# gaspachoo/EEG2Video

Measured on AMD Instinct MI355X. Metric: 6-frame 288x512 clips/sec (50-step DDIM), higher is better.
Workload: dtype f32; 1 GPU; 1xMI355X: batch=8/GPU synthetic latents [B,4,6,36,64] + [B,77,768] cond, 50-step DDIM, CFG 12.5, 288x512x6 VAE decode, fp32 (BASELINE configs[1]); clips_per_gpu=8, ddim_steps=50, unet_samples_per_ddim_step=16, weights=random-init SD-v1-4 architecture, counter RNG seed 42/43, collective=none

## Files before the change

### eeg2video_amd/csrc/attn.hip

```cpp
#include "h16.h"
#include "kernels.h"
#include "prof.h"
#include "runtime.h"
#include "act_io.h"

#include <cstdlib>
#include <type_traits>

namespace e2v {

typedef float f32x16 __attribute__((ext_vector_type(16)));
typedef float f32x4 __attribute__((ext_vector_type(4)));

struct AttnBlock { int qb, head, sf; bool valid; };
__host__ __device__ __forceinline__ int attn_xcd_unit(const int n, const int F, const int heads) {
    return n % 8 == 0 ? 0 : (n * F) % 8 == 0 ? 1 : 2;
}
__device__ __forceinline__ AttnBlock attn_block_of(const AttnArgs& p, const int nqb) {
    const int b = blockIdx.x, xcd = b & 7, idx = b >> 3;
    const int S = p.n * p.F;
    const int unit = attn_xcd_unit(p.n, p.F, p.heads);
    AttnBlock r;
    if (unit == 0) {
        const int per = p.F * p.heads * nqb;
        const int ul = idx / per, w = idx - ul * per;
        const int smp = ul * 8 + xcd;
        const int f = w / (p.heads * nqb), w2 = w - f * (p.heads * nqb);
        r.sf = smp * p.F + f; r.head = w2 / nqb; r.qb = w2 - r.head * nqb; r.valid = smp < p.n;
    } else if (unit == 1) {
        const int per = p.heads * nqb;
        const int ul = idx / per, w = idx - ul * per;
        r.sf = ul * 8 + xcd; r.head = w / nqb; r.qb = w - r.head * nqb; r.valid = r.sf < S;
    } else {
        const int ul = idx / nqb;
        const int pair = ul * 8 + xcd;
        r.qb = idx - ul * nqb; r.sf = pair / p.heads; r.head = pair - r.sf * p.heads; r.valid = pair < S * p.heads;
    }
    return r;
}
__device__ __forceinline__ AttnBlock attn_block(const AttnArgs& p) { return attn_block_of(p, (p.Nq + 127) / 128); }
static inline unsigned attn_grid_of(const AttnArgs& a, const unsigned nqb) {
    const int unit = attn_xcd_unit(a.n, a.F, a.heads);
    if (unit == 0) return 8u * (a.n / 8) * (unsigned)(a.F * a.heads) * nqb;
    if (unit == 1) return 8u * ((a.n * a.F) / 8) * (unsigned)a.heads * nqb;
    return 8u * ((a.n * a.F * a.heads + 7) / 8) * nqb;
}
static inline unsigned attn_grid(const AttnArgs& a) { return attn_grid_of(a, (a.Nq + 127) / 128); }

std::string attn_shape_tag(const AttnArgs& a) {
    return " D" + std::to_string(a.D) + " Nq" + std::to_string(a.Nq) + " Nk" + std::to_string(a.Nk) + " n" + std::to_string(a.n) + " F" + std::to_string(a.F) +
           " h" + std::to_string(a.heads);
}

template <int D>
__global__ __launch_bounds__(256) void flash_attn_kernel(const AttnArgs p) {
    constexpr int LD = D + 4;
    constexpr int TF = D / 32;
    constexpr bool VREM = (D - 32 * TF) == 8;
    constexpr int T = VREM ? TF : (D + 31) / 32;
    constexpr int TA = T > 0 ? T : 1;
    constexpr int G = D / 8;
    constexpr int DQ = D / 4;
    constexpr int KT = 32;
    constexpr int NF4 = KT * DQ;
    constexpr int LPT = (NF4 + 255) / 256;
    extern __shared__ __attribute__((aligned(16))) float smem[];

    const int tid = threadIdx.x;
    const int lane = tid & 63, wave = tid >> 6;
    const int j = lane & 31, h = lane >> 5;
    const AttnBlock blk = attn_block(p);
    if (!blk.valid) return;
    const int sf = blk.sf;
    const int smp = sf / p.F, f = sf - smp * p.F;
    const int head = blk.head;
    const int q0 = (blk.qb * 4 + wave) * 32;
    const bool active = q0 < p.Nq;

    int nseg = 1;
    size_t kvbase[2];
    if (p.mode == 0) {
        kvbase[0] = (size_t)(smp * p.F) * p.Nk;
        kvbase[1] = (size_t)(smp * p.F + (f > 0 ? f - 1 : 0)) * p.Nk;
        nseg = f >= 2 ? 2 : 1;
    } else {
        kvbase[0] = kvbase[1] = (size_t)smp * p.Nk;
    }
    const int tps = (p.Nk + KT - 1) / KT;
    const int ntiles = nseg * tps;

    f32x4 qf[G];
    {
        const int qrow = min(q0 + j, p.Nq - 1);
        const float* qp = p.q + ((size_t)sf * p.Nq + qrow) * p.ldq + head * D + h * 4;
        const float c = p.scale * 1.44269504088896340736f;
#pragma unroll
        for (int g = 0; g < G; ++g) {
            qf[g] = *reinterpret_cast<const f32x4*>(qp + g * 8);
            qf[g] *= c;
        }
    }

    constexpr unsigned OOB = 0x80000000u;
    auto rsrc_of = [](const void* ptr) {
        const unsigned long long v = reinterpret_cast<unsigned long long>(ptr);
        const unsigned lo = __builtin_amdgcn_readfirstlane((unsigned)v);
        const unsigned hi = __builtin_amdgcn_readfirstlane((unsigned)(v >> 32));
        return __builtin_amdgcn_make_buffer_rsrc(reinterpret_cast<void*>(((unsigned long long)hi << 32) | lo), (short)0, 0x7FFFFFF0,
                                                 0x00020000);
    };
    int ld_row[LPT];
    unsigned ld_off[LPT];
#pragma unroll
    for (int e = 0; e < LPT; ++e) {
        const int idx = tid + 256 * e;
        const int row = idx / DQ, c4 = idx - row * DQ;
        ld_row[e] = row;
        ld_off[e] = idx < NF4 ? (unsigned)(row * p.ldkv + c4 * 4) * 4u : OOB;
    }
    f32x4 kreg[LPT], vreg[LPT];
    auto load_tile = [&](int tt) {
        const int seg = tt / tps;
        const int key0 = (tt - seg * tps) * KT;
        const size_t first = (kvbase[seg] + key0) * p.ldkv + head * D;
        const __amdgpu_buffer_rsrc_t rk = rsrc_of(p.k + first), rv = rsrc_of(p.v + first);
        const int left = p.Nk - key0;
#pragma unroll
        for (int e = 0; e < LPT; ++e) {
            unsigned off = ld_off[e];
            if (left < KT) off = ld_row[e] < left ? off : OOB;
            kreg[e] = __builtin_bit_cast(f32x4, __builtin_amdgcn_raw_buffer_load_b128(rk, off, 0, 0));
            vreg[e] = __builtin_bit_cast(f32x4, __builtin_amdgcn_raw_buffer_load_b128(rv, off, 0, 0));
        }
    };
    auto store_tile = [&](int buf) {
        float* Ks = smem + buf * (2 * KT * LD);
        float* Vs = Ks + KT * LD;
#pragma unroll
        for (int e = 0; e < LPT; ++e) {
            const int idx = tid + 256 * e;
            if (idx < NF4) {
                const int row = idx / DQ, c4 = idx - row * DQ;
                *reinterpret_cast<f32x4*>(Ks + row * LD + c4 * 4) = kreg[e];
                *reinterpret_cast<f32x4*>(Vs + row * LD + c4 * 4) = vreg[e];
            }
        }
    };

    f32x16 acc[TA];
#pragma unroll
    for (int t = 0; t < TA; ++t)
#pragma unroll
        for (int r = 0; r < 16; ++r) acc[t][r] = 0.f;
    f32x4 rem0 = {0.f, 0.f, 0.f, 0.f}, rem1 = {0.f, 0.f, 0.f, 0.f};
    float m_i = -INFINITY, l_i = 0.f;

    load_tile(0);
    store_tile(0);
    __syncthreads();

    for (int tt = 0; tt < ntiles; ++tt) {
        const int buf = tt & 1;
        if (tt + 1 < ntiles) load_tile(tt + 1);
        const int seg_c = tt / tps;
        const int kbase = (tt - seg_c * tps) * KT;
        auto tile_body = [&](const int key0, const int sub, auto ragged) {
            const float* Ks = smem + buf * (2 * KT * LD) + sub * 32 * LD;
            const float* Vs = smem + buf * (2 * KT * LD) + KT * LD + sub * 32 * LD;
            const f32x16 zero16 = {0.f, 0.f, 0.f, 0.f, 0.f, 0.f, 0.f, 0.f, 0.f, 0.f, 0.f, 0.f, 0.f, 0.f, 0.f, 0.f};
            f32x16 st;
            const float* kp = Ks + j * LD + h * 4;
#pragma unroll
            for (int g = 0; g < G; ++g) {
                const f32x4 kf = *reinterpret_cast<const f32x4*>(kp + g * 8);
#pragma unroll
                for (int s = 0; s < 4; ++s)
                    st = __builtin_amdgcn_mfma_f32_32x32x2f32(kf[s], qf[g][s], (g == 0 && s == 0) ? zero16 : st, 0, 0, 0);
            }
            if constexpr (decltype(ragged)::value) {
#pragma unroll
                for (int r = 0; r < 16; ++r) {
                    const int key = key0 + (r & 3) + 8 * (r >> 2) + 4 * h;
                    if (key >= p.Nk) st[r] = -INFINITY;
                }
            }
            float mt = st[0];
#pragma unroll
            for (int r = 1; r < 16; ++r) mt = __builtin_fmaxf(mt, st[r]);
            mt = __builtin_fmaxf(mt, __shfl_xor(mt, 32));
            const float m_new = __builtin_fmaxf(m_i, mt);
            const bool moved = __any(m_new > m_i);
            float ps = 0.f;
#pragma unroll
            for (int r = 0; r < 16; ++r) {
                st[r] = __builtin_amdgcn_exp2f(st[r] - m_new);
                ps += st[r];
            }
            float alpha = 1.0f;
            if (moved) {
                alpha = __builtin_amdgcn_exp2f(m_i - m_new);
                l_i *= alpha;
            }
            l_i += ps;
            m_i = m_new;
#pragma unroll
            for (int t = 0; t < T; ++t) {
                if (moved) {
#pragma unroll
                    for (int r = 0; r < 16; ++r) acc[t][r] *= alpha;
                }
                const int dv = min(t * 32 + j, D - 1);
                const float* vp = Vs + (4 * h) * LD + dv;
#pragma unroll
                for (int r = 0; r < 16; ++r) {
                    const float vv = vp[((r & 3) + 8 * (r >> 2)) * LD];
                    acc[t] = __builtin_amdgcn_mfma_f32_32x32x2f32(vv, st[r], acc[t], 0, 0, 0);
                }
            }
            if constexpr (VREM) {
                if (moved) {
                    rem0 *= alpha;
                    rem1 *= alpha;
                }
                const float* vr = Vs + (4 * h) * LD + 32 * TF;
#pragma unroll
                for (int r = 0; r < 16; ++r) {
                    const float* row = vr + ((r & 3) + 8 * (r >> 2)) * LD;
                    const f32x4 v0 = *reinterpret_cast<const f32x4*>(row);
                    const f32x4 v1 = *reinterpret_cast<const f32x4*>(row + 4);
                    rem0 += v0 * st[r];
                    rem1 += v1 * st[r];
                }
            }
        };
#pragma unroll
        for (int sub = 0; sub < KT / 32; ++sub) {
            const int key0 = kbase + 32 * sub;
            if (active && key0 < p.Nk) {
                if (key0 + 32 <= p.Nk) tile_body(key0, sub, std::false_type{});
                else tile_body(key0, sub, std::true_type{});
            }
        }
        if (tt + 1 < ntiles) store_tile(buf ^ 1);
        __syncthreads();
    }

    const float l_tot = l_i + __shfl_xor(l_i, 32);
    if constexpr (VREM) {
#pragma unroll
        for (int e = 0; e < 4; ++e) {
            rem0[e] += __shfl_xor(rem0[e], 32);
            rem1[e] += __shfl_xor(rem1[e], 32);
        }
    }
    if (active && q0 + j < p.Nq) {
        const float inv = 1.0f / l_tot;
        float* op = p.o + ((size_t)sf * p.Nq + q0 + j) * p.ldo + head * D;
#pragma unroll
        for (int t = 0; t < T; ++t)
#pragma unroll
            for (int rg = 0; rg < 4; ++rg) {
                const int dv = t * 32 + 8 * rg + 4 * h;
                if (dv < D) {
                    f32x4 o;
#pragma unroll
                    for (int e = 0; e < 4; ++e) o[e] = acc[t][rg * 4 + e] * inv;
                    *reinterpret_cast<f32x4*>(op + dv) = o;
                }
            }
        if constexpr (VREM) {
            const f32x4 o = (h ? rem1 : rem0) * inv;
            *reinterpret_cast<f32x4*>(op + 32 * TF + 4 * h) = o;
        }
    }
}

typedef __bf16 abf16x4 __attribute__((ext_vector_type(4)));
typedef __bf16 abf16x8 __attribute__((ext_vector_type(8)));

template <typename H, int D, bool FOLD, int KT>
__global__ __launch_bounds__(256) void flash_attn_b16io_kernel(const AttnArgs p) {
    constexpr int DP = (D + 15) / 16 * 16;
    constexpr int KS = DP / 16;
    constexpr int T = (D + 31) / 32;
    constexpr int KROW = DP * 2 + 16;
    constexpr int VROW = ((T * 16) % 32 == 16) ? T * 64 : T * 64 + 64;
    constexpr int KBYTES = KT * KROW, VBYTES = KT * VROW;
    constexpr int STAGE = (KBYTES + VBYTES + 15) / 16 * 16;
    constexpr bool SUMV = (D % 32) != 0;
    constexpr int LROW = D % 32, LREG = 4 * (LROW / 8) + (LROW & 3), LHALF = (LROW >> 2) & 1;
    constexpr int C8 = D / 8;
    constexpr int NP = KT * C8;
    constexpr int LPT = (NP + 255) / 256;
    extern __shared__ __attribute__((aligned(16))) char smem_h[];

    const int tid = threadIdx.x;
    const int lane = tid & 63, wave = tid >> 6;
    const int j = lane & 31, h = lane >> 5;
    const AttnBlock blk = attn_block(p);
    if (!blk.valid) return;
    const int sf = blk.sf;
    const int smp = sf / p.F, f = sf - smp * p.F;
    const int head = blk.head;
    const int q0 = (blk.qb * 4 + wave) * 32;
    const bool active = q0 < p.Nq;
    const H* __restrict__ Q = reinterpret_cast<const H*>(p.q);
    const H* __restrict__ K = reinterpret_cast<const H*>(p.k);
    const H* __restrict__ V = reinterpret_cast<const H*>(p.v);

    int nseg = 1;
    size_t kvbase[2];
    if (p.mode == 0) {
        kvbase[0] = (size_t)(smp * p.F) * p.Nk;
        kvbase[1] = (size_t)(smp * p.F + (f > 0 ? f - 1 : 0)) * p.Nk;
        nseg = f >= 2 ? 2 : 1;
    } else {
        kvbase[0] = kvbase[1] = (size_t)smp * p.Nk;
    }
    const int tps = (p.Nk + KT - 1) / KT;
    const int ntiles = nseg * tps;

    for (int i = tid * 16; i < 2 * STAGE; i += 256 * 16)
        *reinterpret_cast<f32x4*>(smem_h + i) = f32x4{0.f, 0.f, 0.f, 0.f};
    if constexpr (SUMV) {
        __syncthreads();
        if (tid < 2 * KT)
            *reinterpret_cast<H*>(smem_h + (tid / KT) * STAGE + KBYTES + (tid % KT) * VROW + D * 2) = (H)1.0f;
    }

    hx8<H> qf[KS];
    {
        const int qrow = min(q0 + j, p.Nq - 1);
        const H* qp = Q + ((size_t)sf * p.Nq + qrow) * p.ldq + head * D;
#pragma unroll
        for (int s = 0; s < KS; ++s) {
            const int k0 = 16 * s + 8 * h;
            hx8<H> a;
#pragma unroll
            for (int e = 0; e < 8; ++e) a[e] = (H)0.f;
            if (k0 < D) a = *reinterpret_cast<const hx8<H>*>(qp + k0);
            if constexpr (FOLD) {
                const float qs = p.scale * 1.44269504088896340736f;
#pragma unroll
                for (int e = 0; e < 8; ++e) a[e] = (H)((float)a[e] * qs);
            }
            qf[s] = a;
        }
    }
    const float sc = p.scale * 1.44269504088896340736f;
    __syncthreads();

    constexpr unsigned OOB = 0x80000000u;
    auto rsrc_of = [](const void* ptr) {
        const unsigned long long v = reinterpret_cast<unsigned long long>(ptr);
        const unsigned lo = __builtin_amdgcn_readfirstlane((unsigned)v);
        const unsigned hi = __builtin_amdgcn_readfirstlane((unsigned)(v >> 32));
        return __builtin_amdgcn_make_buffer_rsrc(reinterpret_cast<void*>(((unsigned long long)hi << 32) | lo), (short)0, 0x7FFFFFF0,
                                                 0x00020000);
    };
    int ld_row[LPT], ld_c8[LPT];
    unsigned ld_off[LPT];
#pragma unroll
    for (int e = 0; e < LPT; ++e) {
        const int idx = tid + 256 * e;
        const int row = idx / C8, c8 = idx - row * C8;
        ld_row[e] = row; ld_c8[e] = c8;
        ld_off[e] = idx < NP ? (unsigned)(row * p.ldkv + c8 * 8) * 2u : OOB;
    }
    f32x4 kreg[LPT], vreg[LPT];
    auto load_tile = [&](const int seg, const int key0) {
        const size_t first = (kvbase[seg] + key0) * p.ldkv + head * D;
        const __amdgpu_buffer_rsrc_t rk = rsrc_of(K + first), rv = rsrc_of(V + first);
        const int left = p.Nk - key0;
#pragma unroll
        for (int e = 0; e < LPT; ++e) {
            unsigned off = ld_off[e];
            if (left < KT) off = ld_row[e] < left ? off : OOB;
            kreg[e] = __builtin_bit_cast(f32x4, __builtin_amdgcn_raw_buffer_load_b128(rk, off, 0, 0));
            vreg[e] = __builtin_bit_cast(f32x4, __builtin_amdgcn_raw_buffer_load_b128(rv, off, 0, 0));
        }
    };
    auto store_tile = [&](int buf) {
        char* Kl = smem_h + buf * STAGE;
        char* Vl = Kl + KBYTES;
#pragma unroll
        for (int e = 0; e < LPT; ++e) {
            if (tid + 256 * e < NP) {
                *reinterpret_cast<f32x4*>(Kl + ld_row[e] * KROW + ld_c8[e] * 16) = kreg[e];
                *reinterpret_cast<f32x4*>(Vl + ld_row[e] * VROW + ld_c8[e] * 16) = vreg[e];
            }
        }
    };

    f32x16 acc[T];
#pragma unroll
    for (int t = 0; t < T; ++t)
#pragma unroll
        for (int r = 0; r < 16; ++r) acc[t][r] = 0.f;
    float m_i = -INFINITY, l_i = 0.f;
    f32x16 negm;
#pragma unroll
    for (int r = 0; r < 16; ++r) negm[r] = 0.f;

    load_tile(0, 0);
    store_tile(0);
    __syncthreads();

    const int ti = lane & 15;
    const int tr_off = (4 * h + (ti >> 2)) * VROW + (16 * ((lane >> 4) & 1) + 4 * (ti & 3)) * 2;

    int key0 = 0;
    for (int tt = 0; tt < ntiles; ++tt) {
        const int buf = tt & 1;
        if (tt == tps) key0 = 0;
        if (tt + 1 < ntiles) {
            if (tt + 1 == tps) load_tile(1, 0); else load_tile(tt + 1 > tps ? 1 : 0, key0 + KT);
        }
#pragma unroll
        for (int sub = 0; sub < KT / 32; ++sub) {
        const int keyb = key0 + 32 * sub;
        if (active && keyb < p.Nk) {
            const char* Kl = smem_h + buf * STAGE + sub * 32 * KROW;
            const char* Vl = smem_h + buf * STAGE + KBYTES + sub * 32 * VROW;
            const f32x16 zero16 = {0.f, 0.f, 0.f, 0.f, 0.f, 0.f, 0.f, 0.f, 0.f, 0.f, 0.f, 0.f, 0.f, 0.f, 0.f, 0.f};
            f32x16 st;
            const char* kp = Kl + j * KROW + h * 16;
#pragma unroll
            for (int s = 0; s < KS; ++s) {
                const hx8<H> kf = *reinterpret_cast<const hx8<H>*>(kp + s * 32);
                st = mfma_32x32x16(kf, qf[s], s == 0 ? (FOLD ? negm : zero16) : st);
            }
            if (keyb + 32 > p.Nk) {
                asm volatile("" ::: "memory");
#pragma unroll
                for (int r = 0; r < 16; ++r) {
                    const int key = keyb + (r & 3) + 8 * (r >> 2) + 4 * h;
                    if (key >= p.Nk) st[r] = -INFINITY;
                }
            }
            float mt = st[0];
#pragma unroll
            for (int r = 1; r < 16; ++r) mt = __builtin_fmaxf(mt, st[r]);
            float alpha = 1.0f;
            bool moved;
            if constexpr (FOLD) {
                {
                    float a = mt, b = mt;
                    asm volatile("s_nop 1\n\tv_permlane32_swap_b32 %0, %1" : "+v"(a), "+v"(b));
                    mt = __builtin_fmaxf(a, b);
                }
                constexpr float DEFER = 8.0f;
                const bool first = tt == 0 && sub == 0;
                const float d = first ? mt : (mt > DEFER ? mt : 0.f);
                moved = __any(d != 0.f);
                if (moved) {
                    asm volatile("" ::: "memory");
                    alpha = first ? 1.0f : __builtin_amdgcn_exp2f(-d);
#pragma unroll
                    for (int r = 0; r < 16; ++r) { st[r] -= d; negm[r] -= d; }
                }
#pragma unroll
                for (int r = 0; r < 16; ++r) st[r] = __builtin_amdgcn_exp2f(st[r]);
            } else {
                mt = __builtin_fmaxf(mt, __shfl_xor(mt, 32)) * sc;
                const float m_new = __builtin_fmaxf(m_i, mt);
                moved = __any(m_new > m_i);
                float ps = 0.f;
#pragma unroll
                for (int r = 0; r < 16; ++r) {
                    st[r] = __builtin_amdgcn_exp2f(__builtin_fmaf(st[r], sc, -m_new));
                    if constexpr (!SUMV) ps += st[r];
                }
                if (moved) {
                    alpha = __builtin_amdgcn_exp2f(m_i - m_new);
                    if constexpr (!SUMV) l_i *= alpha;
                }
                if constexpr (!SUMV) l_i += ps;
                m_i = m_new;
            }
            if constexpr (FOLD && !SUMV) {
                float ps = 0.f;
#pragma unroll
                for (int r = 0; r < 16; ++r) ps += st[r];
                l_i = l_i * alpha + ps;
            }
            hx8<H> pf[2];
#pragma unroll
            for (int s = 0; s < 2; ++s)
#pragma unroll
                for (int e = 0; e < 8; ++e) pf[s][e] = (H)st[8 * s + e];
#pragma unroll
            for (int t = 0; t < T; ++t) {
                if (moved) {
                    asm volatile("" ::: "memory");
#pragma unroll
                    for (int r = 0; r < 16; ++r) acc[t][r] *= alpha;
                }
                const char* vb = Vl + tr_off + t * 64;
#pragma unroll
                for (int s = 0; s < 2; ++s) {
                    const hx4<H> lo = lds_read_tr16<H>((vb + (16 * s) * VROW));
                    const hx4<H> hi = lds_read_tr16<H>((vb + (16 * s + 8) * VROW));
                    const hx8<H> vf = __builtin_shufflevector(lo, hi, 0, 1, 2, 3, 4, 5, 6, 7);
                    acc[t] = mfma_32x32x16(vf, pf[s], acc[t]);
                }
            }
        }
        }
        if (tt + 1 < ntiles) store_tile(buf ^ 1);
        __syncthreads();
        key0 += KT;
    }

    float l_tot;
    if constexpr (SUMV) l_tot = __shfl(acc[T - 1][LREG], j + 32 * LHALF);
    else l_tot = l_i + __shfl_xor(l_i, 32);
    if (active && q0 + j < p.Nq) {
        const float inv = 1.0f / l_tot;
        H* op = reinterpret_cast<H*>(p.o) + ((size_t)sf * p.Nq + q0 + j) * p.ldo + head * D;
#pragma unroll
        for (int t = 0; t < T; ++t)
#pragma unroll
            for (int rg = 0; rg < 4; ++rg) {
                const int dv = t * 32 + 8 * rg + 4 * h;
                if (dv < D) {
                    hx4<H> o;
#pragma unroll
                    for (int e = 0; e < 4; ++e) o[e] = (H)(acc[t][rg * 4 + e] * inv);
                    *reinterpret_cast<hx4<H>*>(op + dv) = o;
                }
            }
    }
}

template <typename H, int D>
__global__ __launch_bounds__(256) void cross_attn_resident_kernel(const AttnArgs p, const int tpw, const int chunks) {
    constexpr int DP = (D + 15) / 16 * 16;
    constexpr int KS = DP / 16;
    constexpr int T = (D + 31) / 32;
    constexpr int KROW = DP * 2 + 16;
    constexpr int VROW = ((T * 16) % 32 == 16) ? T * 64 : T * 64 + 64;
    constexpr int NKT = 3, NKEY = 32 * NKT;
    constexpr int KBYTES = NKEY * KROW;
    constexpr bool SUMV = (D % 32) != 0;
    constexpr int LROW = D % 32, LREG = 4 * (LROW / 8) + (LROW & 3), LHALF = (LROW >> 2) & 1;
    constexpr int C8 = D / 8;
    extern __shared__ __attribute__((aligned(16))) char smem_c[];

    const int tid = threadIdx.x;
    const int lane = tid & 63, wave = tid >> 6;
    const int j = lane & 31, h = lane >> 5;
    const int b = blockIdx.x, xcd = b & 7, idx = b >> 3;
    int smp, head, chunk;
    if (p.n % 8 == 0) {
        const int per = p.heads * chunks;
// ... 1126 lines not shown
```

Baseline: 0.5995 clips/s.

## Restructure flash-attention tile loop and use permlane swaps and MFMA for remainder

Reworks the flash-attention main loop so buffer indices are compile-time constant in an unrolled pair of steps, and tracks segment and key offsets incrementally instead of dividing each iteration. Replaces cross-half __shfl_xor reductions with v_permlane32_swap via inline asm, hoists the alpha rescale into a single branch, and computes the D%32==8 remainder with 4x4x1 MFMAs instead of vector FMAs. The aim is to cut per-tile index arithmetic, LDS-based shuffles and VALU work. The inline asm relies on gfx950-specific permlane semantics, and the 4x4 MFMA remainder mapping must match the original output layout.

```diff
diff --git a/eeg2video_amd/csrc/attn.hip b/eeg2video_amd/csrc/attn.hip
--- a/eeg2video_amd/csrc/attn.hip
+++ b/eeg2video_amd/csrc/attn.hip
@@ -52,6 +52,11 @@
            " h" + std::to_string(a.heads);
 }
 
+__device__ __forceinline__ void half_pair(const float x, float& lo, float& hi) {
+    lo = x; hi = x;
+    asm volatile("s_nop 1\n\tv_permlane32_swap_b32 %0, %1" : "+v"(lo), "+v"(hi));
+}
+
 template <int D>
 __global__ __launch_bounds__(256) void flash_attn_kernel(const AttnArgs p) {
     constexpr int LD = D + 4;
@@ -119,9 +124,7 @@
         ld_off[e] = idx < NF4 ? (unsigned)(row * p.ldkv + c4 * 4) * 4u : OOB;
     }
     f32x4 kreg[LPT], vreg[LPT];
-    auto load_tile = [&](int tt) {
-        const int seg = tt / tps;
-        const int key0 = (tt - seg * tps) * KT;
+    auto load_tile = [&](const int seg, const int key0) {
         const size_t first = (kvbase[seg] + key0) * p.ldkv + head * D;
         const __amdgpu_buffer_rsrc_t rk = rsrc_of(p.k + first), rv = rsrc_of(p.v + first);
         const int left = p.Nk - key0;
@@ -155,102 +158,120 @@
     f32x4 rem0 = {0.f, 0.f, 0.f, 0.f}, rem1 = {0.f, 0.f, 0.f, 0.f};
     float m_i = -INFINITY, l_i = 0.f;
 
-    load_tile(0);
+    auto tile_body = [&](const int buf, const int key0, const bool ragged) {
+        const float* Ks = smem + buf * (2 * KT * LD);
+        const float* Vs = Ks + KT * LD;
+        const f32x16 zero16 = {0.f, 0.f, 0.f, 0.f, 0.f, 0.f, 0.f, 0.f, 0.f, 0.f, 0.f, 0.f, 0.f, 0.f, 0.f, 0.f};
+        f32x16 st;
+        const float* kp = Ks + j * LD + h * 4;
+#pragma unroll
+        for (int g = 0; g < G; ++g) {
+            const f32x4 kf = *reinterpret_cast<const f32x4*>(kp + g * 8);
+#pragma unroll
+            for (int s = 0; s < 4; ++s)
+                st = __builtin_amdgcn_mfma_f32_32x32x2f32(kf[s], qf[g][s], (g == 0 && s == 0) ? zero16 : st, 0, 0, 0);
+        }
+        if (ragged) {
+            asm volatile("" ::: "memory");
+#pragma unroll
+            for (int r = 0; r < 16; ++r) {
+                const int key = key0 + (r & 3) + 8 * (r >> 2) + 4 * h;
+                if (key >= p.Nk) st[r] = -INFINITY;
+            }
+        }
+        float mt = st[0];
+#pragma unroll
+        for (int r = 1; r < 16; ++r) mt = __builtin_fmaxf(mt, st[r]);
+        {
+            float lo, hi;
+            half_pair(mt, lo, hi);
+            mt = __builtin_fmaxf(lo, hi);
+        }
+        const float m_new = __builtin_fmaxf(m_i, mt);
+        const bool moved = __any(m_new > m_i);
+        float ps = 0.f;
+#pragma unroll
+        for (int r = 0; r < 16; ++r) {
+            st[r] = __builtin_amdgcn_exp2f(st[r] - m_new);
+            ps += st[r];
+        }
+        if (moved) {
+            asm volatile("" ::: "memory");
+            const float alpha = __builtin_amdgcn_exp2f(m_i - m_new);
+            l_i *= alpha;
+#pragma unroll
+            for (int t = 0; t < T; ++t)
+#pragma unroll
+                for (int r = 0; r < 16; ++r) acc[t][r] *= alpha;
+            if constexpr (VREM) {
+                rem0 *= alpha;
+                rem1 *= alpha;
+            }
+        }
+        l_i += ps;
+        m_i = m_new;
+#pragma unroll
+        for (int t = 0; t < T; ++t) {
+            const int dv = min(t * 32 + j, D - 1);
+            const float* vp = Vs + (4 * h) * LD + dv;
+#pragma unroll
+            for (int r = 0; r < 16; ++r) {
+                const float vv = vp[((r & 3) + 8 * (r >> 2)) * LD];
+                acc[t] = __builtin_amdgcn_mfma_f32_32x32x2f32(vv, st[r], acc[t], 0, 0, 0);
+            }
+        }
+        if constexpr (VREM) {
+            const float* vr = Vs + (4 * h) * LD + 32 * TF + (lane & 3);
+#pragma unroll
+            for (int r = 0; r < 16; ++r) {
+                const float* row = vr + ((r & 3) + 8 * (r >> 2)) * LD;
+                rem0 = __builtin_amdgcn_mfma_f32_4x4x1f32(row[0], st[r], rem0, 0, 0, 0);
+                rem1 = __builtin_amdgcn_mfma_f32_4x4x1f32(row[4], st[r], rem1, 0, 0, 0);
+            }
+        }
+    };
+
+    load_tile(0, 0);
     store_tile(0);
     __syncthreads();
 
-    for (int tt = 0; tt < ntiles; ++tt) {
-        const int buf = tt & 1;
-        if (tt + 1 < ntiles) load_tile(tt + 1);
-        const int seg_c = tt / tps;
-        const int kbase = (tt - seg_c * tps) * KT;
-        auto tile_body = [&](const int key0, const int sub, auto ragged) {
-            const float* Ks = smem + buf * (2 * KT * LD) + sub * 32 * LD;
-            const float* Vs = smem + buf * (2 * KT * LD) + KT * LD + sub * 32 * LD;
-            const f32x16 zero16 = {0.f, 0.f, 0.f, 0.f, 0.f, 0.f, 0.f, 0.f, 0.f, 0.f, 0.f, 0.f, 0.f, 0.f, 0.f, 0.f};
-            f32x16 st;
-            const float* kp = Ks + j * LD + h * 4;
-#pragma unroll
-            for (int g = 0; g < G; ++g) {
-                const f32x4 kf = *reinterpret_cast<const f32x4*>(kp + g * 8);
-#pragma unroll
-                for (int s = 0; s < 4; ++s)
-                    st = __builtin_amdgcn_mfma_f32_32x32x2f32(kf[s], qf[g][s], (g == 0 && s == 0) ? zero16 : st, 0, 0, 0);
-            }
-            if constexpr (decltype(ragged)::value) {
-#pragma unroll
-                for (int r = 0; r < 16; ++r) {
-                    const int key = key0 + (r & 3) + 8 * (r >> 2) + 4 * h;
-                    if (key >= p.Nk) st[r] = -INFINITY;
-                }
-            }
-            float mt = st[0];
-#pragma unroll
-            for (int r = 1; r < 16; ++r) mt = __builtin_fmaxf(mt, st[r]);
-            mt = __builtin_fmaxf(mt, __shfl_xor(mt, 32));
-            const float m_new = __builtin_fmaxf(m_i, mt);
-            const bool moved = __any(m_new > m_i);
-            float ps = 0.f;
-#pragma unroll
-            for (int r = 0; r < 16; ++r) {
-                st[r] = __builtin_amdgcn_exp2f(st[r] - m_new);
-                ps += st[r];
-            }
-            float alpha = 1.0f;
-            if (moved) {
-                alpha = __builtin_amdgcn_exp2f(m_i - m_new);
-                l_i *= alpha;
-            }
-            l_i += ps;
-            m_i = m_new;
-#pragma unroll
-            for (int t = 0; t < T; ++t) {
-                if (moved) {
-#pragma unroll
-                    for (int r = 0; r < 16; ++r) acc[t][r] *= alpha;
-                }
-                const int dv = min(t * 32 + j, D - 1);
-                const float* vp = Vs + (4 * h) * LD + dv;
-#pragma unroll
-                for (int r = 0; r < 16; ++r) {
-                    const float vv = vp[((r & 3) + 8 * (r >> 2)) * LD];
-                    acc[t] = __builtin_amdgcn_mfma_f32_32x32x2f32(vv, st[r], acc[t], 0, 0, 0);
-                }
-            }
-            if constexpr (VREM) {
-                if (moved) {
-                    rem0 *= alpha;
-                    rem1 *= alpha;
-                }
-                const float* vr = Vs + (4 * h) * LD + 32 * TF;
-#pragma unroll
-                for (int r = 0; r < 16; ++r) {
-                    const float* row = vr + ((r & 3) + 8 * (r >> 2)) * LD;
-                    const f32x4 v0 = *reinterpret_cast<const f32x4*>(row);
-                    const f32x4 v1 = *reinterpret_cast<const f32x4*>(row + 4);
-                    rem0 += v0 * st[r];
-                    rem1 += v1 * st[r];
-                }
-            }
-        };
-#pragma unroll
-        for (int sub = 0; sub < KT / 32; ++sub) {
-            const int key0 = kbase + 32 * sub;
-            if (active && key0 < p.Nk) {
-                if (key0 + 32 <= p.Nk) tile_body(key0, sub, std::false_type{});
-                else tile_body(key0, sub, std::true_type{});
-            }
-        }
-        if (tt + 1 < ntiles) store_tile(buf ^ 1);
+    const int nfull = p.Nk / KT;
+    int seg = 0, lt = 0;
+    auto step = [&](const int buf, const bool last, const bool ragged) {
+        const int key0 = lt * KT;
+        if (++lt == tps) { lt = 0; ++seg; }
+        if (!last) load_tile(seg, lt * KT);
+        if (active) tile_body(buf, key0, ragged);
+        if (!last) store_tile(buf ^ 1);
         __syncthreads();
-    }
-
-    const float l_tot = l_i + __shfl_xor(l_i, 32);
+    };
+    int tt = 0;
+    while (tt < ntiles) {
+        if (!(tt & 1))
+            for (; tt < ntiles && lt + 2 <= nfull; tt += 2) {
+                step(0, false, false);
+                step(1, tt + 2 == ntiles, false);
+            }
+        if (tt < ntiles) {
+            step(tt & 1, tt + 1 == ntiles, lt >= nfull);
+            ++tt;
+        }
+    }
+
+    float l_tot;
+    {
+        float lo, hi;
+        half_pair(l_i, lo, hi);
+        l_tot = lo + hi;
+    }
     if constexpr (VREM) {
 #pragma unroll
         for (int e = 0; e < 4; ++e) {
-            rem0[e] += __shfl_xor(rem0[e], 32);
-            rem1[e] += __shfl_xor(rem1[e], 32);
+            float lo, hi;
+            half_pair(rem0[e], lo, hi);
+            rem0[e] = lo + hi;
+            half_pair(rem1[e], lo, hi);
+            rem1[e] = lo + hi;
         }
     }
     if (active && q0 + j < p.Nq) {
```

Measured after the change: 0.6101 clips/s (median of 6 runs). 1.8% higher.
